# lz4/lz4-java

Hardware: NVIDIA H100
Metric: lz4_fast_compress_plus_decompress_64KiB_blocks (higher is better)
Workload: dtype u8

## Files before the change

### lz4-java_b200/csrc/lz4_decompress.cu

```cuda
#include "common.cuh"
#include "kernels.h"

namespace b200 {

#ifndef B200_DEC_MINB_BATCH
#define B200_DEC_MINB_BATCH 8
#endif
#ifndef B200_DEC_WIN
#define B200_DEC_WIN 512
#endif
static constexpr int DEC_WIN = B200_DEC_WIN;

struct VarLen { uint32_t len; int ip; bool err; };

__device__ __forceinline__ VarLen read_varlen(const uint8_t* __restrict__ src, int ip, int ilimit, bool initial_check)
{
    VarLen r; r.len = 0; r.ip = ip; r.err = false;
    if (initial_check && ip >= ilimit) { r.err = true; return r; }
    uint32_t s;
    do {
        s = src[r.ip]; r.ip++;
        r.len = min(r.len + s, 0x40000000u);
        if (r.ip > ilimit) { r.err = true; return r; }
    } while (s == 255);
    return r;
}

__device__ __forceinline__ void lane_copy16(uint8_t* d, const uint8_t* s, int n)
{
    const uintptr_t sa = reinterpret_cast<uintptr_t>(s);
    const uint32_t* w = reinterpret_cast<const uint32_t*>(sa & ~uintptr_t(3));
    const uint32_t sh = (uint32_t(sa) & 3u) * 8u;
    uint32_t x[5];
    #pragma unroll
    for (int t = 0; t < 5; t++) x[t] = (4 * t < n + 3) ? w[t] : 0u;
    #pragma unroll
    for (int t = 0; t < 4; t++) {
        const uint32_t v = __funnelshift_r(x[t], x[t + 1], sh);
        if (4 * t     < n) d[4 * t]     = uint8_t(v);
        if (4 * t + 1 < n) d[4 * t + 1] = uint8_t(v >> 8);
        if (4 * t + 2 < n) d[4 * t + 2] = uint8_t(v >> 16);
        if (4 * t + 3 < n) d[4 * t + 3] = uint8_t(v >> 24);
    }
}

__device__ __forceinline__ int decode_batch(const uint8_t* __restrict__ src, uint8_t* dst, int& ip, int& op,
                                            const int iend, const int oend, const int lane, uint8_t* win)
{
    const uint8_t* __restrict__ in = src + ip;
    uint8_t* cls = win + DEC_WIN;
    {
        const uintptr_t base = reinterpret_cast<uintptr_t>(in);
        const uint32_t* __restrict__ W = reinterpret_cast<const uint32_t*>(base & ~uintptr_t(3)) + 4 * lane;
        const uint32_t a8 = (uint32_t(base) & 3u) * 8u;
        const uint32_t w0 = W[0], w1 = W[1], w2 = W[2], w3 = W[3], w4 = W[4];
        uint32_t f[4];
        f[0] = __funnelshift_r(w0, w1, a8); f[1] = __funnelshift_r(w1, w2, a8); f[2] = __funnelshift_r(w2, w3, a8); f[3] = __funnelshift_r(w3, w4, a8);
        uint32_t c[4];
        #pragma unroll
        for (int k = 0; k < 4; k++) {
            const uint32_t t = f[k];
            const uint32_t lit = (t >> 4) & 0x0F0F0F0Fu, ml = t & 0x0F0F0F0Fu;
            const uint32_t m15 = ((ml + 0x01010101u) >> 4) & 0x01010101u;
            c[k] = (lit + 0x03030303u) | (m15 << 5);
        }
        __syncwarp();
        reinterpret_cast<uint4*>(win)[lane] = make_uint4(f[0], f[1], f[2], f[3]);
        reinterpret_cast<uint4*>(cls)[lane] = make_uint4(c[0], c[1], c[2], c[3]);
        __syncwarp();
    }
    auto wbyte = [&](int p) -> uint32_t { return p < DEC_WIN ? win[p] : in[p]; };
    const int ilim = iend - ip - 64;
    const int olim = oend - op - 128;

    int k = 0, q = 0;
    int m_tok = 0;
    while (k < 32 && q < DEC_WIN - 8) {
        const int c = cls[q];
        int s = c & 31;
        if (c > 17) {
            bool ok = true;
            if (s == 18) {
                int p = q + 1, lit = 15; uint32_t e;
                do { if (p >= ilim) { ok = false; break; } e = wbyte(p++); lit += int(e); } while (e == 255u && lit < (1 << 24));
                s = (p - q) + lit + 2;
                ok = ok && lit < (1 << 24);
            }
            if (ok && (c & 32)) {
                uint32_t e; int cnt = 0;
                do { if (q + s >= ilim) { ok = false; break; } e = wbyte(q + s); s++; } while (e == 255u && ++cnt < (1 << 16));
                ok = ok && cnt < (1 << 16);
            }
            if (!ok || q + s > ilim) break;
        }
        if (lane == k) m_tok = q;
        q += s; k++;
    }
    if (k == 0) return 0;
    int m_lit = 0, m_ml = 0, m_lsrc = 0;
    if (lane < k) {
        const uint32_t tok = win[m_tok];
        m_lit = int(tok >> 4); m_ml = int(tok & 15u) + 4; m_lsrc = m_tok + 1;
        if (m_lit == 15) { uint32_t e; do { e = wbyte(m_lsrc++); m_lit += int(e); } while (e == 255u); }
        if (m_ml == 19) { int p = m_lsrc + m_lit + 2; uint32_t e; do { e = wbyte(p++); m_ml += int(e); } while (e == 255u); }
    }
    int m_out = m_lit + m_ml;
    #pragma unroll
    for (int d = 1; d < 32; d <<= 1) { const int y = __shfl_up_sync(B200_FULL, m_out, d); if (lane >= d) m_out += y; }
    {
        const unsigned over = __ballot_sync(B200_FULL, lane < k && m_out > olim);
        if (over) {
            k = __ffs(over) - 1;
            if (k == 0) return 0;
            q = __shfl_sync(B200_FULL, m_tok, k);
        }
    }
    int acc = __shfl_sync(B200_FULL, m_out, k - 1);
    m_out -= m_lit + m_ml;
    if (lane >= k) { m_lit = 0; m_ml = 0; }

    int off = 1;
    if (lane < k) off = int(in[m_lsrc + m_lit]) | (int(in[m_lsrc + m_lit + 1]) << 8);
    const int mstart = op + m_out + m_lit;
    const unsigned bad = __ballot_sync(B200_FULL, lane < k && (off == 0 || off > mstart));
    if (bad) {
        k = __ffs(bad) - 1;
        if (k == 0) return 0;
        acc = __shfl_sync(B200_FULL, m_out, k);
        q = __shfl_sync(B200_FULL, m_tok, k);
    }
    const bool mine = lane < k;

    if (mine) lane_copy16(dst + op + m_out, in + m_lsrc, min(m_lit, 16));
    if (__any_sync(B200_FULL, mine && m_lit > 16)) {
        if (mine && m_lit > 16) lane_copy16(dst + op + m_out + 16, in + m_lsrc + 16, min(m_lit - 16, 16));
        for (unsigned lm = __ballot_sync(B200_FULL, mine && m_lit > 32); lm; lm &= lm - 1) {
            const int j = __ffs(lm) - 1;
            const int jo = __shfl_sync(B200_FULL, m_out, j), js = __shfl_sync(B200_FULL, m_lsrc, j), jl = __shfl_sync(B200_FULL, m_lit, j);
            warp_copy(dst + op + jo + 32, in + js + 32, jl - 32, lane);
        }
    }
    __syncwarp();

    const bool ovl = off < m_ml;
    const int mend = mstart - off + m_ml;
    unsigned pend = k == 32 ? B200_FULL : (1u << k) - 1u;
    while (pend) {
        const int fp = __ffs(pend) - 1;
        const int fpm = __shfl_sync(B200_FULL, mstart, fp);
        if (__shfl_sync(B200_FULL, int(ovl), fp)) {
            warp_match_copy(dst + fpm, __shfl_sync(B200_FULL, off, fp), __shfl_sync(B200_FULL, m_ml, fp), lane);
            pend &= pend - 1;
            __syncwarp();
            continue;
        }
        const bool ready = ((pend >> lane) & 1u) && !ovl && (lane == fp || mend <= fpm);
        const unsigned rm = __ballot_sync(B200_FULL, ready);
        if (ready) lane_copy16(dst + mstart, dst + mstart - off, min(m_ml, 16));
        if (__any_sync(B200_FULL, ready && m_ml > 16)) {
            if (ready && m_ml > 16) lane_copy16(dst + mstart + 16, dst + mstart - off + 16, min(m_ml - 16, 16));
            for (unsigned lm = __ballot_sync(B200_FULL, ready && m_ml > 32); lm; lm &= lm - 1) {
                const int j = __ffs(lm) - 1;
                const int jm = __shfl_sync(B200_FULL, mstart, j), jo = __shfl_sync(B200_FULL, off, j), jl = __shfl_sync(B200_FULL, m_ml, j);
                warp_copy(dst + jm + 32, dst + jm - jo + 32, jl - 32, lane);
            }
        }
        pend &= ~rm;
        __syncwarp();
    }
    ip += q; op += acc;
    return k;
}

template <int WARPS, bool BATCH>
__global__ void __launch_bounds__(WARPS * 32, BATCH ? B200_DEC_MINB_BATCH : 2048 / (WARPS * 32))
lz4_decompress_safe_kernel(const uint8_t* __restrict__ src_base, const uint64_t* __restrict__ src_off,
                           const int32_t* __restrict__ src_len,
                           uint8_t* dst_base, const uint64_t* __restrict__ dst_off,
                           const int32_t* __restrict__ dst_cap, int32_t* __restrict__ result, uint32_t n)
{
    __shared__ __align__(16) uint8_t s_win[BATCH ? WARPS : 1][2 * DEC_WIN];
    uint8_t* win = s_win[BATCH ? (threadIdx.x >> 5) : 0];
    const uint32_t b = blockIdx.x * WARPS + (threadIdx.x >> 5);
    if (b >= n) return;
    const int lane = lane_id();
    const uint8_t* __restrict__ src = src_base + src_off[b];
    uint8_t* dst = dst_base + dst_off[b];
    const int iend = src_len[b];
    const int oend = dst_cap[b];
    int ip = 0, op = 0;
    int ret;

    if (oend < 0) { ret = -1; goto done; }
    if (oend == 0) { ret = (iend == 1 && src[0] == 0) ? 0 : -1; goto done; }
    if (iend <= 0) { ret = -1; goto done; }
    {
        bool fastloop = oend >= 64;
        const uint8_t* __restrict__ sl = src + lane;
        uint8_t* dl = dst + lane;
        for (;;) {
            while (BATCH && fastloop && ip + DEC_WIN + 128 <= iend && op + 256 <= oend) { if (decode_batch(src, dst, ip, op, iend, oend, lane, win) == 0) break; }
            while (fastloop && ip + 18 <= iend) {
                const uint32_t token = src[ip];
                const uint32_t lit = token >> 4, mlc = token & 15;
                if (lit == 15 || mlc == 15) break;
                if (lane < lit) dl[op] = sl[ip + 1];
                const int ipo = ip + 1 + (int)lit;
                const uint32_t off = (uint32_t)src[ipo] | ((uint32_t)src[ipo + 1] << 8);
                const int op2 = op + (int)lit, ml = (int)mlc + 4;
                if (op2 + ml >= oend - 64 || off > (uint32_t)op2 || off == 0) break;
                __syncwarp();
                if (off >= (uint32_t)ml) { if (lane < ml) dl[op2] = dl[op2 - (int)off]; }
                else warp_match_copy(dst + op2, (int)off, ml, lane);
                ip = ipo + 2; op = op2 + ml;
            }
            const uint32_t token = src[ip++];
            uint32_t len = token >> 4;
            bool apply_end_rule, shortcut = false;
            if (fastloop) {
                bool leave;
                if (len == 15) {
                    VarLen v = read_varlen(src, ip, iend - 15, true);
                    ip = v.ip; if (v.err) goto error;
                    len += v.len;
                    leave = ((long long)op + len > oend - 32) || ((long long)ip + len > iend - 32);
                } else leave = ip > iend - 17;
                if (leave) fastloop = false;
                apply_end_rule = leave;
            } else {
                shortcut = (len != 15) && (ip < iend - 16) && (op <= oend - 32);
                if (!shortcut && len == 15) {
                    VarLen v = read_varlen(src, ip, iend - 15, true);
                    ip = v.ip; if (v.err) goto error;
                    len += v.len;
                }
                apply_end_rule = !shortcut;
            }
            const long long lcpy = (long long)op + len;
            if (apply_end_rule && (lcpy > oend - 12 || (long long)ip + len > iend - 8)) {
                if ((long long)ip + len != iend || lcpy > oend) goto error;
                warp_copy(dst + op, src + ip, (int)len, lane);
                op += (int)len;
                break;
            }
            warp_copy(dst + op, src + ip, (int)len, lane);
            ip += (int)len; op += (int)len;

            const int off = src[ip] | (src[ip + 1] << 8);
            ip += 2;
            uint32_t ml = token & 15;
            const bool direct = shortcut && ml != 15 && off >= 8 && off <= op;
            if (ml == 15) {
                VarLen v = read_varlen(src, ip, iend - 4, false);
                ip = v.ip; if (v.err) goto error;
                ml += v.len;
            }
            ml += 4;
            if (!direct) {
                if (off > op) goto error;
                const long long mcpy = (long long)op + ml;
                if (fastloop && mcpy >= oend - 64) fastloop = false;
                if (mcpy > oend - 5) goto error;
            }
            __syncwarp();
            if (off == 0) {
                for (int i = lane; i < (int)ml; i += 32) dst[op + i] = 0;
            } else {
                warp_match_copy(dst + op, off, (int)ml, lane);
            }
            op += (int)ml;
        }
        ret = op;
        goto done;
    }
error:
    ret = -ip - 1;
done:
    __syncwarp();
    if (lane == 0) { __threadfence(); result[b] = ret; }
}

template <int WARPS, bool BATCH>
__global__ void __launch_bounds__(WARPS * 32, BATCH ? B200_DEC_MINB_BATCH : 2048 / (WARPS * 32))
lz4_decompress_fast_kernel(const uint8_t* __restrict__ src_base, const uint64_t* __restrict__ src_off,
                           const int32_t* __restrict__ src_avail,
                           uint8_t* dst_base, const uint64_t* __restrict__ dst_off,
                           const int32_t* __restrict__ dst_len, int32_t* __restrict__ result, uint32_t n)
{
    __shared__ __align__(16) uint8_t s_win[BATCH ? WARPS : 1][2 * DEC_WIN];
    uint8_t* win = s_win[BATCH ? (threadIdx.x >> 5) : 0];
    const uint32_t b = blockIdx.x * WARPS + (threadIdx.x >> 5);
    if (b >= n) return;
    const int lane = lane_id();
    const uint8_t* __restrict__ src = src_base + src_off[b];
    uint8_t* dst = dst_base + dst_off[b];
    const int avail = src_avail[b];
    const int oend = dst_len[b];
    int ip = 0, op = 0, ret = -1;

    if (oend < 0) goto done;
    for (;;) {
        while (BATCH && ip + DEC_WIN + 128 <= avail && op + 256 <= oend) { if (decode_batch(src, dst, ip, op, avail, oend, lane, win) == 0) break; }
        {
            const uint8_t* __restrict__ sl = src + lane;
            uint8_t* dl = dst + lane;
            while (ip + 17 <= avail) {
                const uint32_t token = src[ip];
                const uint32_t lit = token >> 4, mlc = token & 15;
                if (lit == 15 || mlc == 15) break;
                const int op2 = op + (int)lit, ml = (int)mlc + 4;
                if (op2 + 23 > oend) break;
                if (lane < lit) dl[op] = sl[ip + 1];
                const int ipo = ip + 1 + (int)lit;
                const uint32_t off = (uint32_t)src[ipo] | ((uint32_t)src[ipo + 1] << 8);
                if (off > (uint32_t)op2 || off == 0) break;
                __syncwarp();
                if (off >= (uint32_t)ml) { if (lane < ml) dl[op2] = dl[op2 - (int)off]; }
                else warp_match_copy(dst + op2, (int)off, ml, lane);
                ip = ipo + 2; op = op2 + ml;
            }
        }
        if (ip >= avail) goto done;
        const uint32_t token = src[ip++];
        uint32_t ll = token >> 4;
        if (ll == 15) {
            uint32_t s;
            do { if (ip >= avail) goto done; s = src[ip++]; ll = min(ll + s, 0x40000000u); } while (s == 255);
        }
        if ((uint32_t)(oend - op) < ll) goto done;
        if ((long long)ip + ll > avail) goto done;
        warp_copy(dst + op, src + ip, (int)ll, lane);
        op += (int)ll; ip += (int)ll;
        if (oend - op < 12) {
            if (op == oend) { ret = ip; }
            goto done;
        }
        if (ip + 2 > avail) goto done;
        const int off = src[ip] | (src[ip + 1] << 8);
        ip += 2;
        uint32_t ml = token & 15;
        if (ml == 15) {
            uint32_t s;
            do { if (ip >= avail) goto done; s = src[ip++]; ml = min(ml + s, 0x40000000u); } while (s == 255);
        }
        ml += 4;
        if ((uint32_t)(oend - op) < ml) goto done;
        if (off > op) goto done;
        __syncwarp();
        if (off != 0) warp_match_copy(dst + op, off, (int)ml, lane);
        else for (int i = lane; i < (int)ml; i += 32) dst[op + i] = 0;
        op += (int)ml;
        if (oend - op < 5) goto done;
    }
done:
    if (lane == 0) result[b] = ret;
}

#ifndef B200_HOST_SIM
static constexpr int DEC_WARPS = 4;

cudaError_t launch_decompress_safe(const BatchArgs& a, cudaStream_t st)
{
    if (a.n == 0) return cudaSuccess;
    const unsigned grid = (unsigned)((a.n + DEC_WARPS - 1) / DEC_WARPS);
    lz4_decompress_safe_kernel<DEC_WARPS, true><<<grid, DEC_WARPS * 32, 0, st>>>(
        a.src_base, a.src_off, a.src_len, a.dst_base, a.dst_off, a.dst_cap, a.result, (uint32_t)a.n);
    return cudaGetLastError();
}

cudaError_t launch_decompress_fast(const BatchArgs& a, cudaStream_t st)
{
    if (a.n == 0) return cudaSuccess;
    const unsigned grid = (unsigned)((a.n + DEC_WARPS - 1) / DEC_WARPS);
    lz4_decompress_fast_kernel<DEC_WARPS, true><<<grid, DEC_WARPS * 32, 0, st>>>(
        a.src_base, a.src_off, a.src_len, a.dst_base, a.dst_off, a.dst_cap, a.result, (uint32_t)a.n);
    return cudaGetLastError();
}

#endif

}
```

Baseline: 76.76.

## Stage batch output in shared memory and flush with aligned 16-byte stores

Decoded output of each warp batch is built in a per-warp shared-memory staging buffer, reading match sources through a view that spans global and staged bytes. It is then written to global memory as aligned uint4 stores, replacing scattered byte stores. Staging is chosen once per block from the literal-to-output ratio of the first batch, and literal copies now read from the shared window when the bytes fit. Optional clock64 tracing is added under a compile flag. The cost is more shared memory per warp (about 2 KiB extra), which may lower occupancy, plus extra shared-memory traffic and more complex match-copy paths.

```diff
diff --git a/lz4-java_b200/csrc/lz4_decompress.cu b/lz4-java_b200/csrc/lz4_decompress.cu
--- a/lz4-java_b200/csrc/lz4_decompress.cu
+++ b/lz4-java_b200/csrc/lz4_decompress.cu
@@ -10,6 +10,41 @@
 #define B200_DEC_WIN 512
 #endif
 static constexpr int DEC_WIN = B200_DEC_WIN;
+#ifndef B200_DEC_STAGE
+#define B200_DEC_STAGE 2048
+#endif
+#ifndef B200_DEC_STAGE_LIT
+#define B200_DEC_STAGE_LIT 4
+#endif
+static constexpr int DEC_STAGE = B200_DEC_STAGE;
+
+enum { DT_STAGE, DT_WALK, DT_DECODE, DT_LIT, DT_MATCH, DT_FLUSH, DT_SEQ, DT_BATCHES, DT_SEQUENCES, DT_ROUNDS, DT_FALLBACKS,
+       DT_N };
+#ifdef B200_DEC_TRACE
+constexpr int DEC_TRACE_EVERY = 64, DEC_TRACE_ROWS = 16384;
+__device__ unsigned long long g_dec_trace[DEC_TRACE_ROWS][DT_N];
+__device__ __forceinline__ long long dec_clock() { return clock64(); }
+struct DecTrace {
+    unsigned long long* row; long long t;
+    __device__ explicit DecTrace(uint32_t b)
+        : row(b % DEC_TRACE_EVERY == 0 && b / DEC_TRACE_EVERY < DEC_TRACE_ROWS ? g_dec_trace[b / DEC_TRACE_EVERY] : nullptr),
+          t(dec_clock()) {}
+    __device__ void mark(int slot)
+    {
+        if (!row) return;
+        const long long now = dec_clock();
+        if (lane_id() == 0) atomicAdd(row + slot, (unsigned long long)(now - t));
+        t = now;
+    }
+    __device__ void count(int slot, int n = 1) { if (row && lane_id() == 0) atomicAdd(row + slot, (unsigned long long)n); }
+};
+#else
+struct DecTrace {
+    __device__ explicit DecTrace(uint32_t) {}
+    __device__ void mark(int) {}
+    __device__ void count(int, int = 1) {}
+};
+#endif
 
 struct VarLen { uint32_t len; int ip; bool err; };
 
@@ -26,14 +61,8 @@
     return r;
 }
 
-__device__ __forceinline__ void lane_copy16(uint8_t* d, const uint8_t* s, int n)
-{
-    const uintptr_t sa = reinterpret_cast<uintptr_t>(s);
-    const uint32_t* w = reinterpret_cast<const uint32_t*>(sa & ~uintptr_t(3));
-    const uint32_t sh = (uint32_t(sa) & 3u) * 8u;
-    uint32_t x[5];
-    #pragma unroll
-    for (int t = 0; t < 5; t++) x[t] = (4 * t < n + 3) ? w[t] : 0u;
+__device__ __forceinline__ void store16(uint8_t* d, const uint32_t (&x)[5], uint32_t sh, int n)
+{
     #pragma unroll
     for (int t = 0; t < 4; t++) {
         const uint32_t v = __funnelshift_r(x[t], x[t + 1], sh);
@@ -44,16 +73,112 @@
     }
 }
 
+__device__ __forceinline__ void lane_copy16(uint8_t* d, const uint8_t* s, int n)
+{
+    const uintptr_t sa = reinterpret_cast<uintptr_t>(s);
+    const uint32_t* w = reinterpret_cast<const uint32_t*>(sa & ~uintptr_t(3));
+    uint32_t x[5];
+    #pragma unroll
+    for (int t = 0; t < 5; t++) x[t] = (4 * t < n + 3) ? w[t] : 0u;
+    store16(d, x, (uint32_t(sa) & 3u) * 8u, n);
+}
+
+template <bool STAGED>
+struct OutView {
+    const uint8_t* dst; const uint8_t* ob; int sb;
+    __device__ const uint8_t* at(int p) const { return STAGED && p >= sb ? ob + (p - sb) : dst + p; }
+};
+
+template <bool STAGED>
+__device__ __forceinline__ void out_copy16(uint8_t* d, const OutView<STAGED>& v, int p, int n)
+{
+    const uint32_t a = uint32_t(reinterpret_cast<uintptr_t>(v.dst + p)) & 3u;
+    const int w0 = p - int(a);
+    uint32_t x[5];
+    #pragma unroll
+    for (int t = 0; t < 5; t++) x[t] = (4 * t < n + 3) ? *reinterpret_cast<const uint32_t*>(v.at(w0 + 4 * t)) : 0u;
+    store16(d, x, a * 8u, n);
+}
+
+struct BatchSeq { int m_out, m_lsrc, m_lit, m_ml, off, mstart, k; };
+
+template <bool STAGED>
+__device__ __forceinline__ void copy_batch(uint8_t* o, const OutView<STAGED> v, const uint8_t* __restrict__ in, const uint8_t* win,
+                                           const int op, const int lane, const BatchSeq& bs, DecTrace& tr)
+{
+    const int m_out = bs.m_out, m_lsrc = bs.m_lsrc, m_lit = bs.m_lit, m_ml = bs.m_ml, off = bs.off, mstart = bs.mstart, k = bs.k;
+    const bool mine = lane < k;
+    if (mine) lane_copy16(o + m_out, m_lsrc + 16 <= DEC_WIN ? win + m_lsrc : in + m_lsrc, min(m_lit, 16));
+    if (__any_sync(B200_FULL, mine && m_lit > 16)) {
+        if (mine && m_lit > 16) lane_copy16(o + m_out + 16, m_lsrc + 32 <= DEC_WIN ? win + m_lsrc + 16 : in + m_lsrc + 16, min(m_lit - 16, 16));
+        for (unsigned lm = __ballot_sync(B200_FULL, mine && m_lit > 32); lm; lm &= lm - 1) {
+            const int j = __ffs(lm) - 1;
+            const int jo = __shfl_sync(B200_FULL, m_out, j), js = __shfl_sync(B200_FULL, m_lsrc, j), jl = __shfl_sync(B200_FULL, m_lit, j);
+            warp_copy(o + jo + 32, in + js + 32, jl - 32, lane);
+        }
+    }
+    __syncwarp();
+    tr.mark(DT_LIT);
+
+    o -= op;
+    const bool ovl = off < m_ml;
+    const int mend = mstart - off + m_ml;
+    unsigned pend = k == 32 ? B200_FULL : (1u << k) - 1u;
+    while (pend) {
+        tr.count(DT_ROUNDS);
+        const int fp = __ffs(pend) - 1;
+        const int fpm = __shfl_sync(B200_FULL, mstart, fp);
+        if (__shfl_sync(B200_FULL, int(ovl), fp)) {
+            const int jo = __shfl_sync(B200_FULL, off, fp), jl = __shfl_sync(B200_FULL, m_ml, fp);
+            if (!STAGED) {
+                warp_match_copy(o + fpm, jo, jl, lane);
+            } else {
+                int r = lane % jo;
+                const int step = 32 % jo;
+                for (int i = lane; i < jl; i += 32) {
+                    o[fpm + i] = *v.at(fpm - jo + r);
+                    r += step; if (r >= jo) r -= jo;
+                }
+            }
+            pend &= pend - 1;
+            __syncwarp();
+            continue;
+        }
+        const bool ready = ((pend >> lane) & 1u) && !ovl && (lane == fp || mend <= fpm);
+        const unsigned rm = __ballot_sync(B200_FULL, ready);
+        if (ready) out_copy16(o + mstart, v, mstart - off, min(m_ml, 16));
+        if (__any_sync(B200_FULL, ready && m_ml > 16)) {
+            if (ready && m_ml > 16) out_copy16(o + mstart + 16, v, mstart - off + 16, min(m_ml - 16, 16));
+            for (unsigned lm = __ballot_sync(B200_FULL, ready && m_ml > 32); lm; lm &= lm - 1) {
+                const int j = __ffs(lm) - 1;
+                const int jm = __shfl_sync(B200_FULL, mstart, j), jo = __shfl_sync(B200_FULL, off, j), jl = __shfl_sync(B200_FULL, m_ml, j);
+                if (!STAGED || jm - jo + 32 >= v.sb || jm - jo + jl <= v.sb) warp_copy(o + jm + 32, v.at(jm - jo + 32), jl - 32, lane);
+                else for (int i = 32 + lane; i < jl; i += 32) o[jm + i] = *v.at(jm - jo + i);
+            }
+        }
+        pend &= ~rm;
+        __syncwarp();
+    }
+    tr.mark(DT_MATCH);
+
+}
+
 __device__ __forceinline__ int decode_batch(const uint8_t* __restrict__ src, uint8_t* dst, int& ip, int& op,
-                                            const int iend, const int oend, const int lane, uint8_t* win)
+                                            const int iend, const int oend, const int lane, uint8_t* win, int& staged, DecTrace& tr)
 {
     const uint8_t* __restrict__ in = src + ip;
     uint8_t* cls = win + DEC_WIN;
+    uint8_t* ob = win + 2 * DEC_WIN;
+    const int ph = int(reinterpret_cast<uintptr_t>(dst + op) & 15u);
+    const int sb = op - ph;
+    __syncwarp();
     {
         const uintptr_t base = reinterpret_cast<uintptr_t>(in);
         const uint32_t* __restrict__ W = reinterpret_cast<const uint32_t*>(base & ~uintptr_t(3)) + 4 * lane;
         const uint32_t a8 = (uint32_t(base) & 3u) * 8u;
         const uint32_t w0 = W[0], w1 = W[1], w2 = W[2], w3 = W[3], w4 = W[4];
+        const bool head = lane < ph && sb + lane >= 0;
+        const uint8_t h = head ? dst[sb + lane] : 0;
         uint32_t f[4];
         f[0] = __funnelshift_r(w0, w1, a8); f[1] = __funnelshift_r(w1, w2, a8); f[2] = __funnelshift_r(w2, w3, a8); f[3] = __funnelshift_r(w3, w4, a8);
         uint32_t c[4];
@@ -67,8 +192,10 @@
         __syncwarp();
         reinterpret_cast<uint4*>(win)[lane] = make_uint4(f[0], f[1], f[2], f[3]);
         reinterpret_cast<uint4*>(cls)[lane] = make_uint4(c[0], c[1], c[2], c[3]);
+        if (head) ob[lane] = h;
         __syncwarp();
     }
+    tr.mark(DT_STAGE);
     auto wbyte = [&](int p) -> uint32_t { return p < DEC_WIN ? win[p] : in[p]; };
     const int ilim = iend - ip - 64;
     const int olim = oend - op - 128;
@@ -96,6 +223,7 @@
         if (lane == k) m_tok = q;
         q += s; k++;
     }
+    tr.mark(DT_WALK);
     if (k == 0) return 0;
     int m_lit = 0, m_ml = 0, m_lsrc = 0;
     if (lane < k) {
@@ -111,7 +239,7 @@
         const unsigned over = __ballot_sync(B200_FULL, lane < k && m_out > olim);
         if (over) {
             k = __ffs(over) - 1;
-            if (k == 0) return 0;
+            if (k == 0) { tr.mark(DT_DECODE); return 0; }
             q = __shfl_sync(B200_FULL, m_tok, k);
         }
     }
@@ -120,54 +248,36 @@
     if (lane >= k) { m_lit = 0; m_ml = 0; }
 
     int off = 1;
-    if (lane < k) off = int(in[m_lsrc + m_lit]) | (int(in[m_lsrc + m_lit + 1]) << 8);
+    if (lane < k) off = int(wbyte(m_lsrc + m_lit)) | (int(wbyte(m_lsrc + m_lit + 1)) << 8);
     const int mstart = op + m_out + m_lit;
     const unsigned bad = __ballot_sync(B200_FULL, lane < k && (off == 0 || off > mstart));
     if (bad) {
         k = __ffs(bad) - 1;
-        if (k == 0) return 0;
+        if (k == 0) { tr.mark(DT_DECODE); return 0; }
         acc = __shfl_sync(B200_FULL, m_out, k);
         q = __shfl_sync(B200_FULL, m_tok, k);
     }
-    const bool mine = lane < k;
-
-    if (mine) lane_copy16(dst + op + m_out, in + m_lsrc, min(m_lit, 16));
-    if (__any_sync(B200_FULL, mine && m_lit > 16)) {
-        if (mine && m_lit > 16) lane_copy16(dst + op + m_out + 16, in + m_lsrc + 16, min(m_lit - 16, 16));
-        for (unsigned lm = __ballot_sync(B200_FULL, mine && m_lit > 32); lm; lm &= lm - 1) {
-            const int j = __ffs(lm) - 1;
-            const int jo = __shfl_sync(B200_FULL, m_out, j), js = __shfl_sync(B200_FULL, m_lsrc, j), jl = __shfl_sync(B200_FULL, m_lit, j);
-            warp_copy(dst + op + jo + 32, in + js + 32, jl - 32, lane);
-        }
-    }
-    __syncwarp();
-
-    const bool ovl = off < m_ml;
-    const int mend = mstart - off + m_ml;
-    unsigned pend = k == 32 ? B200_FULL : (1u << k) - 1u;
-    while (pend) {
-        const int fp = __ffs(pend) - 1;
-        const int fpm = __shfl_sync(B200_FULL, mstart, fp);
-        if (__shfl_sync(B200_FULL, int(ovl), fp)) {
-            warp_match_copy(dst + fpm, __shfl_sync(B200_FULL, off, fp), __shfl_sync(B200_FULL, m_ml, fp), lane);
-            pend &= pend - 1;
-            __syncwarp();
-            continue;
-        }
-        const bool ready = ((pend >> lane) & 1u) && !ovl && (lane == fp || mend <= fpm);
-        const unsigned rm = __ballot_sync(B200_FULL, ready);
-        if (ready) lane_copy16(dst + mstart, dst + mstart - off, min(m_ml, 16));
-        if (__any_sync(B200_FULL, ready && m_ml > 16)) {
-            if (ready && m_ml > 16) lane_copy16(dst + mstart + 16, dst + mstart - off + 16, min(m_ml - 16, 16));
-            for (unsigned lm = __ballot_sync(B200_FULL, ready && m_ml > 32); lm; lm &= lm - 1) {
-                const int j = __ffs(lm) - 1;
-                const int jm = __shfl_sync(B200_FULL, mstart, j), jo = __shfl_sync(B200_FULL, off, j), jl = __shfl_sync(B200_FULL, m_ml, j);
-                warp_copy(dst + jm + 32, dst + jm - jo + 32, jl - 32, lane);
-            }
-        }
-        pend &= ~rm;
-        __syncwarp();
-    }
+    if (staged < 0) {
+        int lits = m_lit;
+        #pragma unroll
+        for (int d = 16; d > 0; d >>= 1) lits += __shfl_xor_sync(B200_FULL, lits, d);
+        staged = 8 * lits <= B200_DEC_STAGE_LIT * acc;
+    }
+    tr.mark(DT_DECODE);
+    const BatchSeq bs{m_out, m_lsrc, m_lit, m_ml, off, mstart, k};
+    if (staged > 0 && ph + acc <= DEC_STAGE) {
+        copy_batch<true>(ob + ph, OutView<true>{dst, ob, sb}, in, win, op, lane, bs, tr);
+        const int e = ph + acc;
+        const int u0 = sb < 0 ? 1 : 0, u1 = e >> 4;
+        for (int u = u0 + lane; u < u1; u += 32)
+            reinterpret_cast<uint4*>(dst + sb)[u] = reinterpret_cast<const uint4*>(ob)[u];
+        const int j = lane < 16 ? lane : 16 * max(u0, u1) + lane - 16;
+        if (lane < 16 ? (sb < 0 && j >= -sb && j < min(e, 16)) : j < e) dst[sb + j] = ob[j];
+        tr.mark(DT_FLUSH);
+    } else {
+        copy_batch<false>(dst + op, OutView<false>{dst, ob, sb}, in, win, op, lane, bs, tr);
+    }
+    tr.count(DT_BATCHES); tr.count(DT_SEQUENCES, k);
     ip += q; op += acc;
     return k;
 }
@@ -179,7 +289,7 @@
                            uint8_t* dst_base, const uint64_t* __restrict__ dst_off,
                            const int32_t* __restrict__ dst_cap, int32_t* __restrict__ result, uint32_t n)
 {
-    __shared__ __align__(16) uint8_t s_win[BATCH ? WARPS : 1][2 * DEC_WIN];
+    __shared__ __align__(16) uint8_t s_win[BATCH ? WARPS : 1][2 * DEC_WIN + DEC_STAGE + 16];
     uint8_t* win = s_win[BATCH ? (threadIdx.x >> 5) : 0];
     const uint32_t b = blockIdx.x * WARPS + (threadIdx.x >> 5);
     if (b >= n) return;
@@ -190,6 +300,8 @@
     const int oend = dst_cap[b];
     int ip = 0, op = 0;
     int ret;
+    int staged = -1;
+    DecTrace tr(b);
 
     if (oend < 0) { ret = -1; goto done; }
     if (oend == 0) { ret = (iend == 1 && src[0] == 0) ? 0 : -1; goto done; }
@@ -199,7 +311,10 @@
         const uint8_t* __restrict__ sl = src + lane;
         uint8_t* dl = dst + lane;
         for (;;) {
-            while (BATCH && fastloop && ip + DEC_WIN + 128 <= iend && op + 256 <= oend) { if (decode_batch(src, dst, ip, op, iend, oend, lane, win) == 0) break; }
+            tr.mark(DT_SEQ);
+            while (BATCH && fastloop && ip + DEC_WIN + 128 <= iend && op + 256 <= oend) {
+                if (decode_batch(src, dst, ip, op, iend, oend, lane, win, staged, tr) == 0) { tr.count(DT_FALLBACKS); break; }
+            }
             while (fastloop && ip + 18 <= iend) {
                 const uint32_t token = src[ip];
                 const uint32_t lit = token >> 4, mlc = token & 15;
@@ -276,6 +391,7 @@
 error:
     ret = -ip - 1;
 done:
+    tr.mark(DT_SEQ);
     __syncwarp();
     if (lane == 0) { __threadfence(); result[b] = ret; }
 }
@@ -287,7 +403,7 @@
                            uint8_t* dst_base, const uint64_t* __restrict__ dst_off,
                            const int32_t* __restrict__ dst_len, int32_t* __restrict__ result, uint32_t n)
 {
-    __shared__ __align__(16) uint8_t s_win[BATCH ? WARPS : 1][2 * DEC_WIN];
+    __shared__ __align__(16) uint8_t s_win[BATCH ? WARPS : 1][2 * DEC_WIN + DEC_STAGE + 16];
     uint8_t* win = s_win[BATCH ? (threadIdx.x >> 5) : 0];
     const uint32_t b = blockIdx.x * WARPS + (threadIdx.x >> 5);
     if (b >= n) return;
@@ -297,10 +413,15 @@
     const int avail = src_avail[b];
     const int oend = dst_len[b];
     int ip = 0, op = 0, ret = -1;
+    int staged = -1;
+    DecTrace tr(b);
 
     if (oend < 0) goto done;
     for (;;) {
-        while (BATCH && ip + DEC_WIN + 128 <= avail && op + 256 <= oend) { if (decode_batch(src, dst, ip, op, avail, oend, lane, win) == 0) break; }
+        tr.mark(DT_SEQ);
+        while (BATCH && ip + DEC_WIN + 128 <= avail && op + 256 <= oend) {
+            if (decode_batch(src, dst, ip, op, avail, oend, lane, win, staged, tr) == 0) { tr.count(DT_FALLBACKS); break; }
+        }
         {
             const uint8_t* __restrict__ sl = src + lane;
             uint8_t* dl = dst + lane;
@@ -353,18 +474,44 @@
         if (oend - op < 5) goto done;
     }
 done:
+    tr.mark(DT_SEQ);
     if (lane == 0) result[b] = ret;
 }
 
 #ifndef B200_HOST_SIM
 static constexpr int DEC_WARPS = 4;
 
+#ifdef B200_DEC_TRACE
+static int g_dec_pad = 0, g_dec_ctas_per_sm = 0;
+extern "C" int b200lz4_dec_trace_read(unsigned long long* host, int rows)
+{
+    if (rows < 0 || rows > DEC_TRACE_ROWS) return -1;
+    return cudaMemcpyFromSymbol(host, g_dec_trace, size_t(rows) * DT_N * sizeof(unsigned long long)) == cudaSuccess ? DT_N : -1;
+}
+extern "C" int b200lz4_dec_trace_clear()
+{
+    void* p = nullptr;
+    if (cudaGetSymbolAddress(&p, g_dec_trace) != cudaSuccess) return -1;
+    return cudaMemset(p, 0, sizeof(g_dec_trace)) == cudaSuccess ? 0 : -1;
+}
+extern "C" void b200lz4_dec_trace_pad(int bytes) { g_dec_pad = bytes; }
+extern "C" int b200lz4_dec_trace_ctas_per_sm() { return g_dec_ctas_per_sm; }
+template <class K> static size_t dec_smem(K k)
+{
+    cudaFuncSetAttribute(k, cudaFuncAttributeMaxDynamicSharedMemorySize, g_dec_pad);
+    cudaOccupancyMaxActiveBlocksPerMultiprocessor(&g_dec_ctas_per_sm, k, DEC_WARPS * 32, g_dec_pad);
+    return size_t(g_dec_pad);
+}
+#else
+template <class K> static size_t dec_smem(K) { return 0; }
+#endif
+
 cudaError_t launch_decompress_safe(const BatchArgs& a, cudaStream_t st)
 {
     if (a.n == 0) return cudaSuccess;
     const unsigned grid = (unsigned)((a.n + DEC_WARPS - 1) / DEC_WARPS);
-    lz4_decompress_safe_kernel<DEC_WARPS, true><<<grid, DEC_WARPS * 32, 0, st>>>(
-        a.src_base, a.src_off, a.src_len, a.dst_base, a.dst_off, a.dst_cap, a.result, (uint32_t)a.n);
+    auto k = lz4_decompress_safe_kernel<DEC_WARPS, true>;
+    k<<<grid, DEC_WARPS * 32, dec_smem(k), st>>>(a.src_base, a.src_off, a.src_len, a.dst_base, a.dst_off, a.dst_cap, a.result, (uint32_t)a.n);
     return cudaGetLastError();
 }
 
@@ -372,8 +519,8 @@
 {
     if (a.n == 0) return cudaSuccess;
     const unsigned grid = (unsigned)((a.n + DEC_WARPS - 1) / DEC_WARPS);
-    lz4_decompress_fast_kernel<DEC_WARPS, true><<<grid, DEC_WARPS * 32, 0, st>>>(
-        a.src_base, a.src_off, a.src_len, a.dst_base, a.dst_off, a.dst_cap, a.result, (uint32_t)a.n);
+    auto k = lz4_decompress_fast_kernel<DEC_WARPS, true>;
+    k<<<grid, DEC_WARPS * 32, dec_smem(k), st>>>(a.src_base, a.src_off, a.src_len, a.dst_base, a.dst_off, a.dst_cap, a.result, (uint32_t)a.n);
     return cudaGetLastError();
 }
 
```

Result: faster. 77.70 (median of 6 runs) (+1.2%).
